# ishine/dmel_codec

Measured on AMD Instinct MI355X. Metric: audio-sec/sec (encode+decode RTF) @24 kHz batch 32, higher is better.
Workload: dtype f32; 1 GPU; cfg2: encode+decode, 24000 Hz, 80 mel, 8 FSQ groups [7, 5, 5], WaveNet 20+20 layers, BigVGAN-base, batch 32 x 1 s per GPU; lanes=3, vocoder_streams=1

## Files before the change

### dmel_codec_amd/csrc/conv_igemm.hip

```cpp
#include "conv.h"
#include "conv_dev.h"
#include "ops.h"
#include <type_traits>

#include <cmath>
#include <cstdlib>

namespace dmel {


template <int WAVES_M, int WAVES_N, int MT, int NT, int MODE, int HALO>
__global__ __launch_bounds__(64 * WAVES_M * WAVES_N) void conv_igemm_kernel(KArgs a) {
  constexpr int BM = WAVES_M * MT * 32, BN = WAVES_N * NT * 32, NW = WAVES_M * WAVES_N;
  constexpr int XS = BN + HALO;
  constexpr int RW = (kCK + NW - 1) / NW;
  constexpr int XC = (XS + 63) / 64;
  extern __shared__ __attribute__((aligned(16))) float smem[];
  float* Xs = smem;

  const int tid = threadIdx.x, lane = tid & 63, wave = tid >> 6;
  const int wave_m = wave / WAVES_N, wave_n = wave % WAVES_N;
  const int h = lane >> 5, l31 = lane & 31;
  int tile_n, mblk, b;
  if (!conv_block_coords(a, tile_n, mblk, b)) return;
  const int q0 = tile_n * BN;
  const int lb = b / a.len_div;

  floatx16 acc[MT][NT];
#pragma unroll
  for (int mi = 0; mi < MT; ++mi)
#pragma unroll
    for (int ni = 0; ni < NT; ++ni)
#pragma unroll
      for (int r = 0; r < 16; ++r) acc[mi][ni][r] = 0.f;

  const float4* wA[MT];
#pragma unroll
  for (int mi = 0; mi < MT; ++mi) {
    const int tile = min(mblk * (BM / 32) + wave_m * MT + mi, a.mtiles - 1);
    wA[mi] = reinterpret_cast<const float4*>(a.w) + (size_t)tile * a.steps * 128 + lane;
  }
  float4 ac0[MT], ac1[MT], an0[MT], an1[MT];
  float xr[RW][XC];

  auto load_x = [&](int sg, int chunk) {
    const float* xb = a.seg[sg].x + (int64_t)b * a.seg[sg].bstride;
    const int taps = a.seg[sg].taps, dil = a.seg[sg].dil, tstride = a.seg[sg].tstride, Cin = a.seg[sg].Cin;
    const int wx = BN + (taps - 1) * dil;
    const int tin = (int)a.seg[sg].Tin;
    const int lim = a.seg[sg].in_len ? min((int)min(a.seg[sg].in_len[lb], (int64_t)tin), tin) : tin;
    const int tau0 = q0 * tstride + a.seg[sg].toff - a.seg[sg].pad_left;
    const int cs = (int)a.seg[sg].cstride;
#pragma unroll
    for (int rr = 0; rr < RW; ++rr) {
      const int r = wave + rr * NW;
      const int ci = chunk * kCK + r;
      const bool rowok = (r < kCK) && (ci < Cin);
      const float* xrow = xb + min(ci, Cin - 1) * cs;
#pragma unroll
      for (int c = 0; c < XC; ++c) {
        const int j = lane + 64 * c;
        const int tau = tau0 + j * tstride;
        const bool ok = rowok && (j < wx) && (tau >= 0) && (tau < lim);
        const float v = xrow[min(max(tau, 0), tin - 1)];
        xr[rr][c] = ok ? v : 0.f;
      }
    }
  };
  auto store_x = [&](float* dst, float scale) {
#pragma unroll
    for (int rr = 0; rr < RW; ++rr) {
      const int r = wave + rr * NW;
#pragma unroll
      for (int c = 0; c < XC; ++c) {
        const int j = lane + 64 * c;
        if ((kCK % NW == 0 || r < kCK) && (XS % 64 == 0 || j < XS)) dst[r * XS + j] = xr[rr][c] * scale;
      }
    }
  };

  int sg = 0, chunk = 0, tap = 0, xbuf = 0;
  load_x(0, 0);
#pragma unroll
  for (int mi = 0; mi < MT; ++mi) { ac0[mi] = wA[mi][0]; ac1[mi] = wA[mi][64]; }
  store_x(Xs, a.seg[0].in_scale);
  __syncthreads();

  for (int s = 0; s < a.steps; ++s) {
    int nsg = sg, nchunk = chunk, ntap = tap + 1;
    bool newx = false;
    if (ntap == a.seg[sg].taps) {
      ntap = 0;
      ++nchunk;
      newx = true;
      if (nchunk == a.seg[sg].nchunk) { nchunk = 0; ++nsg; }
    }
    const bool has_next = s + 1 < a.steps;
    if (has_next) {
#pragma unroll
      for (int mi = 0; mi < MT; ++mi) {
        an0[mi] = wA[mi][(size_t)(s + 1) * 128];
        an1[mi] = wA[mi][(size_t)(s + 1) * 128 + 64];
      }
      if (newx) load_x(nsg, nchunk);
    }
    {
      const float* xp = Xs + xbuf * (kCK * XS) + wave_n * (NT * 32) + l31 + tap * a.seg[sg].dil + h * XS;
#pragma unroll
      for (int kk = 0; kk < kCK / 2; ++kk) {
        float av[MT], bv[NT];
#pragma unroll
        for (int mi = 0; mi < MT; ++mi) {
          const float4 q = (kk < 4) ? ac0[mi] : ac1[mi];
          av[mi] = (kk & 3) == 0 ? q.x : (kk & 3) == 1 ? q.y : (kk & 3) == 2 ? q.z : q.w;
        }
#pragma unroll
        for (int ni = 0; ni < NT; ++ni) bv[ni] = xp[2 * kk * XS + ni * 32];
#pragma unroll
        for (int mi = 0; mi < MT; ++mi)
#pragma unroll
          for (int ni = 0; ni < NT; ++ni)
            acc[mi][ni] = __builtin_amdgcn_mfma_f32_32x32x2f32(av[mi], bv[ni], acc[mi][ni], 0, 0, 0);
      }
    }
    if (has_next) {
#pragma unroll
      for (int mi = 0; mi < MT; ++mi) { ac0[mi] = an0[mi]; ac1[mi] = an1[mi]; }
      if (newx) {
        store_x(Xs + (xbuf ^ 1) * (kCK * XS), a.seg[nsg].in_scale);
        __syncthreads();
        xbuf ^= 1;
      }
    }
    sg = nsg; chunk = nchunk; tap = ntap;
  }

  conv_epilogue<MT, NT, MODE>(a, acc, mblk * BM + wave_m * (MT * 32), q0 + wave_n * (NT * 32) + l31, b, lb, h);
}

template <int WAVES_M, int WAVES_N, int MT, int NT, int MODE>
__global__ __launch_bounds__(64 * WAVES_M * WAVES_N) void conv_direct_kernel(KArgs a) {
  constexpr int BM = WAVES_M * MT * 32, BN = WAVES_N * NT * 32;
  const int tid = threadIdx.x, lane = tid & 63, wave = tid >> 6;
  const int wave_m = wave / WAVES_N, wave_n = wave % WAVES_N;
  const int h = lane >> 5, l31 = lane & 31;
  int tile_n, mblk, b;
  if (!conv_block_coords(a, tile_n, mblk, b)) return;
  const int q0 = tile_n * BN;
  const int lb = b / a.len_div;

  floatx16 acc[MT][NT];
#pragma unroll
  for (int mi = 0; mi < MT; ++mi)
#pragma unroll
    for (int ni = 0; ni < NT; ++ni)
#pragma unroll
      for (int r = 0; r < 16; ++r) acc[mi][ni][r] = 0.f;

  const float4* wA[MT];
#pragma unroll
  for (int mi = 0; mi < MT; ++mi) {
    const int tile = min(mblk * (BM / 32) + wave_m * MT + mi, a.mtiles - 1);
    wA[mi] = reinterpret_cast<const float4*>(a.w) + (size_t)tile * a.steps * 128 + lane;
  }
  const int qcol = q0 + wave_n * (NT * 32) + l31;

  float4 ac0[MT], ac1[MT], an0[MT], an1[MT];
  float bc[NT][8], bn[NT][8];
  int sbase = 0;

  for (int sg = 0; sg < a.nseg; ++sg) {
    const SegArgs& sa = a.seg[sg];
    const float* xb = sa.x + (int64_t)b * sa.bstride;
    const int taps = sa.taps, dil = sa.dil, cin = sa.Cin, cs = (int)sa.cstride, tin = (int)sa.Tin;
    const int lim = sa.in_len ? min((int)min(sa.in_len[lb], (int64_t)tin), tin) : tin;
    const float scale = sa.in_scale;
    const int nst = sa.nchunk * taps;
    int tcol[NT];
#pragma unroll
    for (int ni = 0; ni < NT; ++ni) tcol[ni] = (qcol + ni * 32) * sa.tstride + sa.toff - sa.pad_left;
    int rowoff[8];

#define DMEL_DIRECT_LOAD(A0, A1, B, chunk, tap, gstep)                                                  \
    {                                                                                                   \
      _Pragma("unroll") for (int mi = 0; mi < MT; ++mi) {                                               \
        A0[mi] = wA[mi][(size_t)(gstep) * 128];                                                         \
        A1[mi] = wA[mi][(size_t)(gstep) * 128 + 64];                                                    \
      }                                                                                                 \
      if ((tap) == 0) {                                                                                 \
        _Pragma("unroll") for (int kk = 0; kk < 8; ++kk)                                                \
          rowoff[kk] = min((chunk) * kCK + 2 * kk + h, cin - 1) * cs;                                   \
      }                                                                                                 \
      _Pragma("unroll") for (int ni = 0; ni < NT; ++ni) {                                               \
        const int tau = tcol[ni] + (tap) * dil;                                                         \
        const bool ok = (tau >= 0) && (tau < lim);                                                      \
        const int tc = min(max(tau, 0), tin - 1);                                                       \
        _Pragma("unroll") for (int kk = 0; kk < 8; ++kk) {                                              \
          const float v = xb[rowoff[kk] + tc];                                                          \
          B[ni][kk] = ok ? v * scale : 0.f;                                                             \
        }                                                                                               \
      }                                                                                                 \
    }

    int chunk = 0, tap = 0;
    DMEL_DIRECT_LOAD(ac0, ac1, bc, 0, 0, sbase)
    for (int ls = 0; ls < nst; ++ls) {
      int ntap = tap + 1, nchunk = chunk;
      if (ntap == taps) { ntap = 0; ++nchunk; }
      const bool has_next = ls + 1 < nst;
      if (has_next) DMEL_DIRECT_LOAD(an0, an1, bn, nchunk, ntap, sbase + ls + 1)
#pragma unroll
      for (int kk = 0; kk < 8; ++kk) {
        float av[MT];
#pragma unroll
        for (int mi = 0; mi < MT; ++mi) {
          const float4 q = (kk < 4) ? ac0[mi] : ac1[mi];
          av[mi] = (kk & 3) == 0 ? q.x : (kk & 3) == 1 ? q.y : (kk & 3) == 2 ? q.z : q.w;
        }
#pragma unroll
        for (int mi = 0; mi < MT; ++mi)
#pragma unroll
          for (int ni = 0; ni < NT; ++ni)
            acc[mi][ni] = __builtin_amdgcn_mfma_f32_32x32x2f32(av[mi], bc[ni][kk], acc[mi][ni], 0, 0, 0);
      }
      if (has_next) {
#pragma unroll
        for (int mi = 0; mi < MT; ++mi) { ac0[mi] = an0[mi]; ac1[mi] = an1[mi]; }
#pragma unroll
        for (int ni = 0; ni < NT; ++ni)
#pragma unroll
          for (int kk = 0; kk < 8; ++kk) bc[ni][kk] = bn[ni][kk];
      }
      chunk = nchunk; tap = ntap;
    }
#undef DMEL_DIRECT_LOAD
    sbase += nst;
  }
  conv_epilogue<MT, NT, MODE>(a, acc, mblk * BM + wave_m * (MT * 32), qcol, b, lb, h);
}

static int conv_grid(KArgs& k, int gx, int gy, int gz, dim3& grid) {
  static int mode = [] { const char* e = getenv("DMEL_CONV_XCD"); return e ? atoi(e) : -1; }();
  k.gx = gx; k.gy = gy; k.gz = gz;
  const double weight_bytes = (double)k.mtiles * 32.0 * k.steps * kCK * 4.0;
  const bool want = mode == 1 || (mode == -1 && weight_bytes > 2.5e6 && gy >= 8);
  const int64_t total = (int64_t)gx * gy * gz;
  if (want && total < ((int64_t)1 << 30)) {
    k.xcd_chunk = (int)((total + 7) / 8);
    grid = dim3((unsigned)(k.xcd_chunk * 8));
    return DMEL_OK;
  }
  k.xcd_chunk = 0;
  if (gy > 65535 || gz > 65535) {
    set_error("conv_igemm: grid too large (mblocks %d, batch %d)", gy, gz);
    return DMEL_EINVAL;
  }
  grid = dim3((unsigned)gx, (unsigned)gy, (unsigned)gz);
  return DMEL_OK;
}

template <int WM, int WN, int MT, int NT, int MODE> static int launch_d(const KArgs& ka, int B, int mblocks, hipStream_t st) {
  constexpr int BN = WN * NT * 32;
  KArgs k2 = ka;
  dim3 grid;
  DMEL_TRY(conv_grid(k2, (int)((ka.Tcols + BN - 1) / BN), mblocks, B, grid));
  hipLaunchKernelGGL((conv_direct_kernel<WM, WN, MT, NT, MODE>), grid, dim3(64 * WM * WN), 0, st, k2);
  DMEL_HIP(hipGetLastError());
  return DMEL_OK;
}

template <int WM, int WN, int MT, int NT, int MODE, int HALO>
static int launch_h(const KArgs& ka, int B, int mblocks, hipStream_t st) {
  constexpr int BN = WN * NT * 32;
  const size_t lds = (size_t)(2 * kCK * (BN + HALO)) * sizeof(float);
  KArgs k2 = ka;
  dim3 grid;
  DMEL_TRY(conv_grid(k2, (int)((ka.Tcols + BN - 1) / BN), mblocks, B, grid));
  hipLaunchKernelGGL((conv_igemm_kernel<WM, WN, MT, NT, MODE, HALO>), grid, dim3(64 * WM * WN), lds, st, k2);
  DMEL_HIP(hipGetLastError());
  return DMEL_OK;
}

template <int WM, int WN, int MT, int NT, int MODE> static int launch_t(const KArgs& ka, int B, int mblocks, hipStream_t st) {
  int halo = 0;
  for (int s = 0; s < ka.nseg; ++s) halo = std::max(halo, (ka.seg[s].taps - 1) * ka.seg[s].dil);
  if (halo == 0) return launch_h<WM, WN, MT, NT, MODE, 0>(ka, B, mblocks, st);
  if (halo <= 16) return launch_h<WM, WN, MT, NT, MODE, 16>(ka, B, mblocks, st);
  return launch_h<WM, WN, MT, NT, MODE, 64>(ka, B, mblocks, st);
}

typedef __bf16 bf16x8 __attribute__((ext_vector_type(8)));
typedef _Float16 f16x8 __attribute__((ext_vector_type(8)));
typedef _Float16 f16x2 __attribute__((ext_vector_type(2)));
#ifndef DMEL_PD
#define DMEL_PD 2
#endif
#ifndef DMEL_EXP
#define DMEL_EXP 0
#endif
#ifndef DMEL_PD2
#define DMEL_PD2 2
#endif
#ifndef DMEL_XTOP
#define DMEL_XTOP 0
#endif
#ifndef DMEL_BPF
#define DMEL_BPF 0
#endif
#ifndef DMEL_KG2
#define DMEL_KG2 2
#endif

__device__ __forceinline__ uint32_t pack_hi16(float lo, float hi) {
  return __builtin_amdgcn_perm(__float_as_uint(hi), __float_as_uint(lo), 0x07060302u);
}

template <int WAVES_M, int WAVES_N, int MT, int NT, int MODE, int HALO, int NP, int KG, int PS = 0>
__global__ __launch_bounds__(64 * WAVES_M * WAVES_N, NP == 2 ? 2 : 1) void conv_bf16_kernel(KArgs a) {
  static_assert(PS == 0 || NP == 2, "pre-split inputs exist for the fp16 split only");
  constexpr int BM = WAVES_M * MT * 32, BN = WAVES_N * NT * 32;
  constexpr int XS = BN + HALO;
  constexpr int SUB = KG / 2;
  constexpr int NWV = WAVES_M * WAVES_N;
  static_assert(NWV % KG == 0 || KG % NWV == 0, "waves and staged channel groups must divide one another");
  constexpr int SEG = NWV >= KG ? NWV / KG : 1;
  constexpr int RPW = NWV >= KG ? 1 : KG / NWV;
  constexpr int SL = (XS + SEG - 1) / SEG;
  constexpr int NPASS = (SL + 63) / 64;
  constexpr int NIT = RPW * NPASS;
  constexpr int PSZ = KG * XS;
  extern __shared__ __attribute__((aligned(16))) float smem[];
#ifndef DMEL_CONV_LDS_PAD
#define DMEL_CONV_LDS_PAD 0
#endif
  constexpr int kLdsPad = ((size_t)2 * NP * KG * XS * 16 + 2 * DMEL_CONV_LDS_PAD <= 65536) ? DMEL_CONV_LDS_PAD : 0;
  uint4* Xb = reinterpret_cast<uint4*>(smem) + kLdsPad / 16;

  const int tid = threadIdx.x, lane = tid & 63, wave = tid >> 6;
  const int wave_m = wave / WAVES_N, wave_n = wave % WAVES_N;
  const int h = lane >> 5, l31 = lane & 31;
  int tile_n, mblk, b;
  if (!conv_block_coords(a, tile_n, mblk, b)) return;
  const int q0 = tile_n * BN;
  const int lb = b / a.len_div;

  floatx16 acc[MT][NT];
#pragma unroll
  for (int mi = 0; mi < MT; ++mi)
#pragma unroll
    for (int ni = 0; ni < NT; ++ni)
#pragma unroll
      for (int r = 0; r < 16; ++r) acc[mi][ni][r] = 0.f;
  floatx16 acl[NP == 2 ? MT : 1][NP == 2 ? NT : 1];
  if constexpr (NP == 2) {
#pragma unroll
    for (int mi = 0; mi < MT; ++mi)
#pragma unroll
      for (int ni = 0; ni < NT; ++ni)
#pragma unroll
        for (int r = 0; r < 16; ++r) acl[mi][ni][r] = 0.f;
  }

  const char* wT[MT];
#pragma unroll
  for (int mi = 0; mi < MT; ++mi) {
    const int tile = __builtin_amdgcn_readfirstlane(min(mblk * (BM / 32) + wave_m * MT + mi, a.mtiles - 1));
    wT[mi] = reinterpret_cast<const char*>(NP == 3 ? a.w48 : NP == 2 ? a.w32h : a.w16) + (size_t)tile * a.steps * (NP * 1024);
  }
  const uint32_t lane16 = lane * 16;
  auto load_w = [&](uint4 (&dst)[MT][NP], int step) {
#pragma unroll
    for (int mi = 0; mi < MT; ++mi) {
      const char* sp = wT[mi] + (size_t)step * (NP * 1024);
#pragma unroll
      for (int p = 0; p < NP; ++p) dst[mi][p] = *reinterpret_cast<const uint4*>(sp + p * 1024 + lane16);
    }
  };
  float xr[NIT][8];

  auto seg_limit = [&](int sg) {
    const int tin = (int)a.seg[sg].Tin;
    return a.seg[sg].in_len ? (int)min(a.seg[sg].in_len[lb], (int64_t)tin) : tin;
  };
  const int lim0 = seg_limit(0), lim1 = a.nseg > 1 ? seg_limit(1) : 0;
  float f16_in = kF16XScale, f16_out = 1.f;
  if (NP == 2 && a.seg[0].in_absmax) {
    const int e = min(max((int)(*a.seg[0].in_absmax >> 23) - 127, -100), 100);
    f16_in = __uint_as_float((uint32_t)(127 + 13 - e) << 23);
    f16_out = __uint_as_float((uint32_t)(127 - 13 + e) << 23) * (1.f / kF16WScale);
  }
  bool xok[NIT];
  const int wave_u = __builtin_amdgcn_readfirstlane(wave);
  const int st_kg0 = (wave_u / SEG) * RPW, st_j0 = (wave_u % SEG) * SL;
  auto load_x = [&](int sg, int chunk) {
    if constexpr (PS != 0) {
      const int taps = a.seg[sg].taps, dil = a.seg[sg].dil;
      const int wx = BN + (taps - 1) * dil;
      const int tin = (int)a.seg[sg].Tin, g8 = a.seg[sg].xp_g8;
      const int lim = sg == 0 ? lim0 : lim1;
      const int tau0 = q0 + a.seg[sg].toff - a.seg[sg].pad_left;
      const uint4* xpb = a.seg[sg].xp + (int64_t)b * g8 * tin;
#pragma unroll
      for (int rr = 0; rr < RPW; ++rr) {
        const int kgi = chunk * KG + st_kg0 + rr;
        const uint4* rowp = xpb + (int64_t)min(kgi, g8 - 1) * tin;
#pragma unroll
        for (int ps = 0; ps < NPASS; ++ps) {
          const int it = rr * NPASS + ps;
          const int j = min(st_j0 + ps * 64 + lane, XS - 1);
          const int tau = tau0 + j;
          xok[it] = (j < wx) && (tau >= 0) && (tau < lim) && (kgi < g8);
          const uint4* ptr = rowp + min(max(tau, 0), tin - 1);
          const uint4 hi = *ptr, lo = *(ptr + a.seg[sg].xp_plane);
          xr[it][0] = __uint_as_float(hi.x); xr[it][1] = __uint_as_float(hi.y); xr[it][2] = __uint_as_float(hi.z); xr[it][3] = __uint_as_float(hi.w);
          xr[it][4] = __uint_as_float(lo.x); xr[it][5] = __uint_as_float(lo.y); xr[it][6] = __uint_as_float(lo.z); xr[it][7] = __uint_as_float(lo.w);
        }
      }
      return;
    }
    const char* xb = reinterpret_cast<const char*>(a.seg[sg].x + (int64_t)b * a.seg[sg].bstride);
    const int taps = a.seg[sg].taps, dil = a.seg[sg].dil, tstride = a.seg[sg].tstride, Cin = a.seg[sg].Cin;
    const int wx = BN + (taps - 1) * dil;
    const int tin = (int)a.seg[sg].Tin;
    const int lim = sg == 0 ? lim0 : lim1;
    const int tau0 = q0 * tstride + a.seg[sg].toff - a.seg[sg].pad_left;
    const uint32_t cs4 = (uint32_t)a.seg[sg].cstride * 4u, last = (uint32_t)(Cin - 1) * cs4;
#pragma unroll
    for (int rr = 0; rr < RPW; ++rr) {
      uint32_t row = (uint32_t)(chunk * (KG * 8) + (st_kg0 + rr) * 8) * cs4;
      const char* rowp[8];
#pragma unroll
      for (int e = 0; e < 8; ++e, row += cs4) rowp[e] = xb + min(row, last);
#pragma unroll
      for (int ps = 0; ps < NPASS; ++ps) {
        const int it = rr * NPASS + ps;
        const int j = min(st_j0 + ps * 64 + lane, XS - 1);
        const int tau = tau0 + j * tstride;
        xok[it] = (j < wx) && (tau >= 0) && (tau < lim);
        const uint32_t col = (uint32_t)min(max(tau, 0), tin - 1) * 4u;
#pragma unroll
        for (int e = 0; e < 8; ++e) xr[it][e] = *reinterpret_cast<const float*>(rowp[e] + col);
      }
    }
  };
  auto store_x = [&](uint4* dst, int sg, int chunk) {
#pragma clang fp contract(off)
    if constexpr (PS != 0) {
#pragma unroll
      for (int it = 0; it < NIT; ++it) {
        const int rr = it / NPASS, ps = it % NPASS;
        const int jl = ps * 64 + lane;
        const int j = st_j0 + jl;
        if ((SL % 64 != 0 && jl >= SL) || (XS % SL != 0 && j >= XS)) continue;
        const int i = (st_kg0 + rr) * XS + j;
        const bool ok = xok[it];
        dst[i] = make_uint4(ok ? __float_as_uint(xr[it][0]) : 0u, ok ? __float_as_uint(xr[it][1]) : 0u, ok ? __float_as_uint(xr[it][2]) : 0u,
                            ok ? __float_as_uint(xr[it][3]) : 0u);
        dst[PSZ + i] = make_uint4(ok ? __float_as_uint(xr[it][4]) : 0u, ok ? __float_as_uint(xr[it][5]) : 0u, ok ? __float_as_uint(xr[it][6]) : 0u,
                                  ok ? __float_as_uint(xr[it][7]) : 0u);
      }
      return;
    }
    const float scale = NP == 2 ? a.seg[sg].in_scale * f16_in : a.seg[sg].in_scale;
    const int Cin = a.seg[sg].Cin;
#pragma unroll
    for (int it = 0; it < NIT; ++it) {
      const int rr = it / NPASS, ps = it % NPASS;
      const int jl = ps * 64 + lane;
      const int j = st_j0 + jl;
      if ((SL % 64 != 0 && jl >= SL) || (XS % SL != 0 && j >= XS)) continue;
      const int i = (st_kg0 + rr) * XS + j;
      const int c0 = chunk * (KG * 8) + (st_kg0 + rr) * 8;
      float v[8];
#pragma unroll
      for (int e = 0; e < 8; ++e) v[e] = (xok[it] ? xr[it][e] : 0.f) * (c0 + e < Cin ? scale : 0.f);
      if constexpr (NP == 1) {
        bf16x8 p;
#pragma unroll
        for (int e = 0; e < 8; ++e) p[e] = (__bf16)v[e];
        dst[i] = __builtin_bit_cast(uint4, p);
      } else if constexpr (NP == 2) {
        f16x8 ph, pl;
#pragma unroll
        for (int e = 0; e < 8; e += 2) {
          typedef float f32x2 __attribute__((ext_vector_type(2)));
          const f16x2 hi = __builtin_convertvector((f32x2){v[e], v[e + 1]}, f16x2);
          const f16x2 lo = __builtin_convertvector((f32x2){(v[e] - (float)hi[0]) * kF16LoScale, (v[e + 1] - (float)hi[1]) * kF16LoScale}, f16x2);
          ph[e] = hi[0]; ph[e + 1] = hi[1];
          pl[e] = lo[0]; pl[e + 1] = lo[1];
        }
        dst[i] = __builtin_bit_cast(uint4, ph);
        dst[PSZ + i] = __builtin_bit_cast(uint4, pl);
      } else {
        uint32_t p1[4], p2[4], p3[4];
#pragma unroll
        for (int e = 0; e < 8; e += 2) {
          const float r0 = v[e] - __uint_as_float(__float_as_uint(v[e]) & 0xffff0000u);
          const float r1 = v[e + 1] - __uint_as_float(__float_as_uint(v[e + 1]) & 0xffff0000u);
          const float s0 = r0 - __uint_as_float(__float_as_uint(r0) & 0xffff0000u);
          const float s1 = r1 - __uint_as_float(__float_as_uint(r1) & 0xffff0000u);
          p1[e >> 1] = pack_hi16(v[e], v[e + 1]);
          p2[e >> 1] = pack_hi16(r0, r1);
          p3[e >> 1] = pack_hi16(s0, s1);
        }
        dst[i] = make_uint4(p1[0], p1[1], p1[2], p1[3]);
        dst[PSZ + i] = make_uint4(p2[0], p2[1], p2[2], p2[3]);
        dst[2 * PSZ + i] = make_uint4(p3[0], p3[1], p3[2], p3[3]);
      }
    }
  };
  int cur_taps = a.seg[0].taps, cur_nchunk = a.seg[0].nchunk, cur_dil = a.seg[0].dil;
  auto next_chunk = [&](int sg, int ck, int& nsg, int& nck) -> bool {
    nsg = sg; nck = ck + 1;
    if (nck * SUB >= cur_nchunk) { nck = 0; ++nsg; }
    return nsg < a.nseg;
  };

  int sg = 0, c16 = 0, tap = 0, xbuf = 0;
  int psg = 0, pck = 0;
  bool pending = false;
  constexpr int PD = NP == 2 ? DMEL_PD2 : DMEL_PD;
  uint4 wa[PD + 1][MT][NP];
#pragma unroll
  for (int d = 0; d < PD; ++d) load_w(wa[d], min(d, a.steps - 1));
  load_x(0, 0);
  store_x(Xb, 0, 0);
  __builtin_amdgcn_s_waitcnt(0x0f70);
  __syncthreads();
  int cstep = 0;

  constexpr int kWLoads = MT * NP;
  constexpr int kWKeep = (PD - 1) * kWLoads < 63 ? (PD - 1) * kWLoads : 63;
  constexpr int kWaitW = (kWKeep & 15) | (7 << 4) | (15 << 8) | ((kWKeep >> 4) << 14);
  constexpr int kXLoads = NIT * (PS != 0 ? 2 : 8);
  constexpr int kWX = kWKeep + kXLoads < 63 ? kWKeep + kXLoads : 63;
  [[maybe_unused]] constexpr int kWaitWX = (kWX & 15) | (7 << 4) | (15 << 8) | ((kWX >> 4) << 14);
#if DMEL_BPF
  bf16x8 bfrag[2][NT][NP];
  bool have_frag = false;
#endif
  auto k_step = [&](auto R, int s) {
    constexpr int r = decltype(R)::value;
    uint4 (&use)[MT][NP] = wa[r % (PD + 1)];
    int nsg = sg, nc16 = c16, ntap = tap + 1;
    bool newx = false;
    if (ntap == cur_taps) {
      ntap = 0;
      ++nc16;
      if (nc16 == cur_nchunk) { nc16 = 0; ++nsg; newx = true; }
      else newx = (nc16 % SUB) == 0;
    }
    const bool has_next = s + 1 < a.steps;
#if DMEL_XTOP
    bool x_younger = false;
    if (cstep == 0) {
      pending = next_chunk(sg, c16 / SUB, psg, pck);
      if (pending && !(DMEL_EXP & 2)) { load_x(psg, pck); x_younger = !newx; }
      if (DMEL_EXP & 2) pending = false;
    }
#endif
    if (!(DMEL_EXP & 4)) load_w(wa[(r + PD) % (PD + 1)], min(s + PD, a.steps - 1));
    {
#if DMEL_BPF
      bf16x8 (&bcur)[NT][NP] = bfrag[r % 2];
      bf16x8 (&bnxt)[NT][NP] = bfrag[(r + 1) % 2];
      if (!have_frag) {
        const uint4* xp = Xb + xbuf * (NP * PSZ) + ((c16 % SUB) * 2 + h) * XS + wave_n * (NT * 32) + l31 + tap * cur_dil;
#pragma unroll
        for (int ni = 0; ni < NT; ++ni)
#pragma unroll
          for (int p = 0; p < NP; ++p) bcur[ni][p] = __builtin_bit_cast(bf16x8, xp[p * PSZ + ni * 32]);
      }
      have_frag = has_next && !newx;
      if (have_frag) {
        const uint4* xq = Xb + xbuf * (NP * PSZ) + ((nc16 % SUB) * 2 + h) * XS + wave_n * (NT * 32) + l31 + ntap * cur_dil;
#pragma unroll
        for (int ni = 0; ni < NT; ++ni)
#pragma unroll
          for (int p = 0; p < NP; ++p) bnxt[ni][p] = __builtin_bit_cast(bf16x8, xq[p * PSZ + ni * 32]);
      }
#else
      const uint4* xp = Xb + xbuf * (NP * PSZ) + ((c16 % SUB) * 2 + h) * XS + wave_n * (NT * 32) + l31 + tap * cur_dil;
      bf16x8 bcur[NT][NP];
#pragma unroll
      for (int ni = 0; ni < NT; ++ni)
#pragma unroll
        for (int p = 0; p < NP; ++p) bcur[ni][p] = __builtin_bit_cast(bf16x8, xp[p * PSZ + ni * 32]);
#endif
      if constexpr (NP == 2) {
#pragma unroll
        for (int mi = 0; mi < MT; ++mi)
#pragma unroll
          for (int ni = 0; ni < NT; ++ni) {
            const f16x8 ah = __builtin_bit_cast(f16x8, use[mi][0]), al = __builtin_bit_cast(f16x8, use[mi][1]);
            const f16x8 bh = __builtin_bit_cast(f16x8, bcur[ni][0]), bl = __builtin_bit_cast(f16x8, bcur[ni][1]);
            acl[mi][ni] = __builtin_amdgcn_mfma_f32_32x32x16_f16(ah, bl, acl[mi][ni], 0, 0, 0);
            acl[mi][ni] = __builtin_amdgcn_mfma_f32_32x32x16_f16(al, bh, acl[mi][ni], 0, 0, 0);
            acc[mi][ni] = __builtin_amdgcn_mfma_f32_32x32x16_f16(ah, bh, acc[mi][ni], 0, 0, 0);
          }
      } else {
        constexpr int PA[6] = {2, 1, 0, 1, 0, 0}, PB[6] = {0, 1, 2, 0, 1, 0};
#pragma unroll
        for (int t = 0; t < (NP == 3 ? 6 : 1); ++t)
#pragma unroll
          for (int mi = 0; mi < MT; ++mi)
#pragma unroll
            for (int ni = 0; ni < NT; ++ni)
              acc[mi][ni] = __builtin_amdgcn_mfma_f32_32x32x16_bf16(__builtin_bit_cast(bf16x8, use[mi][NP == 3 ? PA[t] : 0]),
                                                                    bcur[ni][NP == 3 ? PB[t] : 0], acc[mi][ni], 0, 0, 0);
      }
    }
#if DMEL_XTOP
    if (x_younger) __builtin_amdgcn_s_waitcnt(kWaitWX);
    else __builtin_amdgcn_s_waitcnt(kWaitW);
#else
    __builtin_amdgcn_s_waitcnt(kWaitW);
    if (cstep == 0) {
      pending = next_chunk(sg, c16 / SUB, psg, pck);
      if (pending && !(DMEL_EXP & 2)) load_x(psg, pck);
      if (DMEL_EXP & 2) pending = false;
    }
#endif
    if (pending && (((DMEL_EXP & 1) ? false : cstep == 1) || newx)) {
      store_x(Xb + (xbuf ^ 1) * (NP * PSZ), psg, pck);
      pending = false;
    }
    ++cstep;
    if (has_next && newx) {
      __syncthreads();
      xbuf ^= 1;
      cstep = 0;
      if (nsg != sg) { cur_taps = a.seg[nsg].taps; cur_nchunk = a.seg[nsg].nchunk; cur_dil = a.seg[nsg].dil; }
    }
    sg = nsg; c16 = nc16; tap = ntap;
  };
  constexpr int UNR = DMEL_BPF ? ((PD + 1) % 2 ? 2 * (PD + 1) : PD + 1) : PD + 1;
  static_assert(UNR <= 8, "k_step calls below cover an unroll of up to eight");
  for (int s = 0; s < a.steps; s += UNR) {
    k_step(std::integral_constant<int, 0>{}, s);
    if (s + 1 < a.steps) k_step(std::integral_constant<int, 1>{}, s + 1);
    if (UNR > 2 && s + 2 < a.steps) k_step(std::integral_constant<int, 2 % UNR>{}, s + 2);
    if (UNR > 3 && s + 3 < a.steps) k_step(std::integral_constant<int, 3 % UNR>{}, s + 3);
    if (UNR > 4 && s + 4 < a.steps) k_step(std::integral_constant<int, 4 % UNR>{}, s + 4);
    if (UNR > 5 && s + 5 < a.steps) k_step(std::integral_constant<int, 5 % UNR>{}, s + 5);
    if (UNR > 6 && s + 6 < a.steps) k_step(std::integral_constant<int, 6 % UNR>{}, s + 6);
    if (UNR > 7 && s + 7 < a.steps) k_step(std::integral_constant<int, 7 % UNR>{}, s + 7);
  }
  if constexpr (NP == 2) {
#pragma unroll
    for (int mi = 0; mi < MT; ++mi)
#pragma unroll
      for (int ni = 0; ni < NT; ++ni)
#pragma unroll
        for (int r = 0; r < 16; ++r) acc[mi][ni][r] = fmaf(acl[mi][ni][r], 1.f / kF16LoScale, acc[mi][ni][r]) * f16_out;
  }
  if ((DMEL_EXP & 8) && acc[0][0][0] != 12345.f) return;
  conv_epilogue<MT, NT, MODE, NP == 2 ? 8 : 4>(a, acc, mblk * BM + wave_m * (MT * 32), q0 + wave_n * (NT * 32) + l31, b, lb, h);
}

template <int WM, int WN, int MT, int NT, int MODE, int HALO, int NP, int KG, int PS = 0>
static int launch_b16k(const KArgs& ka, int B, int mblocks, hipStream_t st) {
  constexpr int BN = WN * NT * 32;
#ifndef DMEL_CONV_LDS_PAD
#define DMEL_CONV_LDS_PAD 0
#endif
  constexpr size_t lds0 = (size_t)2 * NP * KG * (BN + HALO) * 16;
  constexpr size_t lds = lds0 + (lds0 + 2 * DMEL_CONV_LDS_PAD <= 65536 ? 2 * DMEL_CONV_LDS_PAD : 0);
  static_assert(lds <= 64 * 1024, "bf16 conv tile exceeds the default dynamic LDS limit");
  KArgs k2 = ka;
  dim3 grid;
  DMEL_TRY(conv_grid(k2, (int)((ka.Tcols + BN - 1) / BN), mblocks, B, grid));
  hipLaunchKernelGGL((conv_bf16_kernel<WM, WN, MT, NT, MODE, HALO, NP, KG, PS>), grid, dim3(64 * WM * WN), lds, st, k2);
  DMEL_HIP(hipGetLastError());
  return DMEL_OK;
}

template <int WM, int WN, int MT, int NT, int MODE, int NP> static int launch_b16(const KArgs& ka, int B, int mblocks, hipStream_t st) {
  int halo = 0;
  for (int s = 0; s < ka.nseg; ++s) halo = std::max(halo, (ka.seg[s].taps - 1) * ka.seg[s].dil);
  constexpr int KG0 = (WN * NT * 32 >= 256 && NP == 3) ? 2 : 4;
  if (halo == 0) return launch_b16k<WM, WN, MT, NT, MODE, 0, NP, KG0>(ka, B, mblocks, st);
  constexpr int KGT = (NP == 2 && 2 * NP * DMEL_KG2 * (WN * NT * 32 + 64) * 16 <= 65536) ? DMEL_KG2 : 2;
  if (halo <= 16) return launch_b16k<WM, WN, MT, NT, MODE, 16, NP, KGT>(ka, B, mblocks, st);
  return launch_b16k<WM, WN, MT, NT, MODE, 64, NP, KGT>(ka, B, mblocks, st);
}

#ifndef DMEL_TILE5_NARROW
#define DMEL_TILE5_NARROW 1
#endif
template <int MODE, int NP> static int launch_mode_bf16(const KArgs& ka, int tile, int B, hipStream_t st) {
  const int bm[8] = {128, 128, 64, 32, 128, DMEL_TILE5_NARROW ? 128 : 64, 128, 256};
  const int mblocks = (ka.mtiles * 32 + bm[tile] - 1) / bm[tile];
  switch (tile) {
    case 0: return launch_b16<2, 2, 2, 2, MODE, NP>(ka, B, mblocks, st);
    case 1: return launch_b16<4, 1, 1, 3, MODE, NP>(ka, B, mblocks, st);
    case 2: return launch_b16<2, 2, 1, 2, MODE, NP>(ka, B, mblocks, st);
    case 3: return launch_b16<1, 4, 1, 2, MODE, NP>(ka, B, mblocks, st);
    case 4: return launch_b16<4, 1, 1, 4, MODE, NP>(ka, B, mblocks, st);
    case 6: return launch_b16<4, 1, 1, 2, MODE, NP>(ka, B, mblocks, st);
    case 7: return launch_b16<8, 1, 1, 3, MODE, NP>(ka, B, mblocks, st);
#if DMEL_TILE5_NARROW
    default: return launch_b16<4, 1, 1, 1, MODE, NP>(ka, B, mblocks, st);
#else
    default: return launch_b16<2, 1, 1, 4, MODE, NP>(ka, B, mblocks, st);
#endif
  }
}

static int pick_tile_bf16(int mtiles, int64_t T, int np, int steps, int B) {
  const char* e = getenv("DMEL_CONV_TILE_BF16");
  const int forced = (e && e[0]) ? atoi(e) : -1;
  if (forced >= 0 && forced < 8) return forced;
  int t;
  if (np == 2 && mtiles >= 8 && T > 96) t = 7;
  else if (np == 2 && mtiles >= 4 && mtiles < 8 && steps >= 40) t = 6;
  else if (mtiles >= 4) t = (T > 2048 && np != 2) ? 4 : 1;
  else if (mtiles >= 2) t = 2;
  else t = 3;
  if (np == 2 && mtiles >= 4) {
    static const int bm[8] = {128, 128, 64, 32, 128, DMEL_TILE5_NARROW ? 128 : 64, 128, 256};
    static const int bn[8] = {128, 96, 128, 256, 128, DMEL_TILE5_NARROW ? 32 : 128, 64, 96};
    auto wgs = [&](int tt) { return (int64_t)((mtiles * 32 + bm[tt] - 1) / bm[tt]) * ((T + bn[tt] - 1) / bn[tt]) * B; };
    static const bool off = [] { const char* f = getenv("DMEL_CONV_SMALLN"); return f && f[0] == '0'; }();
    if (!off && wgs(t) < 128) {
      t = 6;
      if (DMEL_TILE5_NARROW && wgs(6) < 128) t = 5;
    }
  }
  return t;
}

template <int MODE> static int launch_presplit(const KArgs& ka, int B, int64_t Tcols, hipStream_t st) {
  int halo = 0;
  for (int s = 0; s < ka.nseg; ++s) halo = std::max(halo, (ka.seg[s].taps - 1) * ka.seg[s].dil);
  if (halo > 16) { set_error("conv (pre-split input): receptive field %d exceeds the 16-column halo built for this path", halo); return DMEL_EUNSUPPORTED; }
  const bool wide = ka.mtiles >= 8 && Tcols > 96;
  if (wide) {
    const int mblocks = (ka.mtiles * 32 + 255) / 256;
    if (halo == 0) return launch_b16k<8, 1, 1, 3, MODE, 0, 2, 4, 1>(ka, B, mblocks, st);
    return launch_b16k<8, 1, 1, 3, MODE, 16, 2, DMEL_KG2, 1>(ka, B, mblocks, st);
  }
  const int mblocks = (ka.mtiles * 32 + 127) / 128;
  if (halo == 0) return launch_b16k<4, 1, 1, 3, MODE, 0, 2, 4, 1>(ka, B, mblocks, st);
  return launch_b16k<4, 1, 1, 3, MODE, 16, 2, DMEL_KG2, 1>(ka, B, mblocks, st);
}

template <int NP> static int launch_bf16_any(const KArgs& ka, EpiMode mode, int B, int64_t Tcols, hipStream_t st) {
  const int t16 = pick_tile_bf16(ka.mtiles, Tcols, NP, ka.steps, B);
  switch (mode) {
    case EPI_LINEAR: return launch_mode_bf16<EPI_LINEAR, NP>(ka, t16, B, st);
    case EPI_GATE: return launch_mode_bf16<EPI_GATE, NP>(ka, t16, B, st);
    default: return launch_mode_bf16<EPI_RESSKIP, NP>(ka, t16, B, st);
  }
}

struct TileCfg {
  int wm, wn, mt, nt;
  float eff;
};
static const TileCfg kTiles[] = {
    {2, 2, 2, 2, 0.93f},
    {4, 1, 1, 3, 1.00f},
    {2, 2, 1, 2, 0.92f},
    {2, 1, 1, 3, 0.85f},
    {1, 4, 1, 2, 0.90f},
    {1, 4, 1, 1, 0.80f},
    {1, 3, 1, 1, 0.80f},
    {1, 4, 1, 1, 0.00f},
    {1, 3, 1, 1, 0.00f},
    {1, 4, 1, 2, 0.00f},
    {2, 2, 1, 2, 0.00f},
    {4, 1, 1, 3, 0.00f},
    {2, 2, 2, 2, 0.00f},
    {2, 2, 1, 1, 0.00f},
};
constexpr int kNumTiles = sizeof(kTiles) / sizeof(kTiles[0]);

static int pick_tile(int mtiles, int64_t T, int B) {
  static int forced = [] {
    const char* e = getenv("DMEL_CONV_TILE");
    return e ? atoi(e) : -1;
  }();
  if (forced >= 0 && forced < kNumTiles) return forced;
  if (T <= 96 && mtiles >= 4) return 8;
  int best = 0;
  double best_cost = 1e300;
  for (int i = 0; i < kNumTiles; ++i) {
    if (kTiles[i].eff <= 0.f) continue;
    const int bm = kTiles[i].wm * kTiles[i].mt * 32, bn = kTiles[i].wn * kTiles[i].nt * 32;
    const double wgs = (double)((mtiles * 32 + bm - 1) / bm) * (double)((T + bn - 1) / bn) * B;
    const double rounds = std::ceil(wgs / 256.0);
    const double cost = (wgs > 1024 ? wgs / 256.0 : rounds) * bm * bn / kTiles[i].eff;
    if (cost < best_cost) { best_cost = cost; best = i; }
  }
  return best;
}

template <int MODE> static int launch_mode(const KArgs& ka, int tile, int B, hipStream_t st) {
  const TileCfg& t = kTiles[tile];
  const int mblocks = (ka.mtiles * 32 + t.wm * t.mt * 32 - 1) / (t.wm * t.mt * 32);
  switch (tile) {
    case 0: return launch_t<2, 2, 2, 2, MODE>(ka, B, mblocks, st);
    case 1: return launch_t<4, 1, 1, 3, MODE>(ka, B, mblocks, st);
    case 2: return launch_t<2, 2, 1, 2, MODE>(ka, B, mblocks, st);
    case 3: return launch_t<2, 1, 1, 3, MODE>(ka, B, mblocks, st);
    case 4: return launch_t<1, 4, 1, 2, MODE>(ka, B, mblocks, st);
    case 5: return launch_t<1, 4, 1, 1, MODE>(ka, B, mblocks, st);
    case 6: return launch_t<1, 3, 1, 1, MODE>(ka, B, mblocks, st);
    case 7: return launch_d<1, 4, 1, 1, MODE>(ka, B, mblocks, st);
    case 8: return launch_d<1, 3, 1, 1, MODE>(ka, B, mblocks, st);
    case 9: return launch_d<1, 4, 1, 2, MODE>(ka, B, mblocks, st);
    case 10: return launch_d<2, 2, 1, 2, MODE>(ka, B, mblocks, st);
    case 11: return launch_d<4, 1, 1, 3, MODE>(ka, B, mblocks, st);
    case 12: return launch_d<2, 2, 2, 2, MODE>(ka, B, mblocks, st);
    default: return launch_d<2, 2, 1, 1, MODE>(ka, B, mblocks, st);
  }
}

__global__ __launch_bounds__(256) void split_planes_kernel(const float* __restrict__ x, uint4* __restrict__ planes, int64_t plane_units,
                                                           const int64_t* __restrict__ len, int len_div, int C, int T) {
  const int b = blockIdx.z, g = blockIdx.y;
  const int t = blockIdx.x * 256 + threadIdx.x;
  if (t >= T) return;
  const float* xr = x + ((int64_t)b * C + g * 8) * T + t;
  const bool live = !len || t < len[b / len_div];
  float v[8];
#pragma unroll
  for (int e = 0; e < 8; ++e) v[e] = live ? xr[(int64_t)e * T] : 0.f;
  f16x8 ph, pl;
  {
#pragma clang fp contract(off)
#pragma unroll
    for (int e = 0; e < 8; e += 2) {
      typedef float f32x2 __attribute__((ext_vector_type(2)));
      const float s0 = v[e] * kF16XScale, s1 = v[e + 1] * kF16XScale;
      const f16x2 hi = __builtin_convertvector((f32x2){s0, s1}, f16x2);
      const f16x2 lo = __builtin_convertvector((f32x2){(s0 - (float)hi[0]) * kF16LoScale, (s1 - (float)hi[1]) * kF16LoScale}, f16x2);
      ph[e] = hi[0]; ph[e + 1] = hi[1];
      pl[e] = lo[0]; pl[e + 1] = lo[1];
    }
  }
  const int64_t i = ((int64_t)b * (C / 8) + g) * T + t;
  planes[i] = __builtin_bit_cast(uint4, ph);
  planes[plane_units + i] = __builtin_bit_cast(uint4, pl);
}
int launch_split_planes(const float* x, void* planes, int64_t plane_units, const int64_t* len, int len_div, int B, int C, int64_t T,
                        hipStream_t stream) {
  DMEL_CHECK_ARG(x && planes && B > 0 && B <= 65535 && C > 0 && C % 8 == 0 && C / 8 <= 65535 && T > 0 && T < ((int64_t)1 << 30), "split_planes: bad argument");
  ProfScope ps("small", stream, 0.0, 8.0 * B * C * (double)T);
  hipLaunchKernelGGL(split_planes_kernel, dim3((unsigned)((T + 255) / 256), (unsigned)(C / 8), (unsigned)B), dim3(256), 0, stream, x,
                     reinterpret_cast<uint4*>(planes), plane_units, len, len_div > 0 ? len_div : 1, C, (int)T);
  DMEL_HIP(hipGetLastError());
  return DMEL_OK;
}

static int check_f16_range(const PackedConv& pc, const ConvRun& r, hipStream_t stream) {
  static const int range_check = [] { const char* e = getenv("DMEL_DEBUG_F16_RANGE"); return e ? atoi(e) : 0; }();
  if (!range_check) return DMEL_OK;
  const PackDesc& d = pc.d;
  for (int s = 0; s < d.nseg; ++s) {
    const SegRun& sr = r.seg[s];
    if (sr.in_absmax || sr.cstride != sr.Tin || sr.bstride != (int64_t)d.seg[s].Cin * sr.cstride) continue;
    const uint32_t* slot = nullptr;
    DMEL_TRY(launch_absmax(sr.x, (int64_t)r.B * sr.bstride, stream, &slot));
    uint32_t bits = 0;
    DMEL_HIP(hipMemcpyAsync(&bits, slot, sizeof(bits), hipMemcpyDeviceToHost, stream));
    DMEL_HIP(hipStreamSynchronize(stream));
    float mx;
    std::memcpy(&mx, &bits, sizeof(mx));
    if (!(mx * sr.in_scale < kF16WScale * 65504.f)) {
      set_error("conv (fp16 split): max |x| = %g of input segment %d is outside the documented domain |x| < %g "
                "(DMEL_PRECISION_FP32_F16X2; use DMEL_PRECISION_FP32_BF16X3 for such tensors)", (double)mx * sr.in_scale, s,
                (double)(kF16WScale * 65504.f));
      return DMEL_EINVAL;
    }
  }
  return DMEL_OK;
}

int launch_conv(const PackedConv& pc, const ConvRun& r, hipStream_t stream) {
  {
    const char* e = getenv("DMEL_CONV_PC");
    if (!(e && e[0] == '0') && conv_pc_eligible(pc, r, e && e[0] == '2')) {
      DMEL_TRY(check_f16_range(pc, r, stream));
      return launch_conv_pc(pc, r, stream);
    }
  }
  KArgs ka{};
  const PackDesc& d = pc.d;
  ka.nseg = d.nseg;
  ka.steps = pc.steps;
  int max_halo = 0;
  for (int s = 0; s < d.nseg; ++s) {
    const SegDesc& sd = d.seg[s];
    SegArgs& o = ka.seg[s];
    DMEL_CHECK_ARG(r.seg[s].x != nullptr || r.seg[s].xp != nullptr, "conv: input pointer of segment %d is NULL", s);
    DMEL_CHECK_ARG(r.seg[s].xp == nullptr || (r.precision == DMEL_PRECISION_FP32_F16X2 && sd.Cin % 8 == 0 && sd.tstride == 1 &&
                                              r.seg[s].in_scale == 1.f && r.seg[s].tshift == 0 && r.seg[s].in_absmax == nullptr && r.fold_pitch == 0),
                   "conv: a pre-split input needs the fp16-split precision, channels %% 8 == 0, unit stride and scale");
    DMEL_CHECK_ARG((r.seg[s].xp != nullptr) == (r.seg[0].xp != nullptr), "conv: either every input segment is pre-split or none is");
    DMEL_CHECK_ARG(sd.taps == 1 || sd.tstride == 1 || (r.precision != DMEL_PRECISION_FP32_MFMA && !getenv("DMEL_CONV_FP32_MFMA")),
                   "conv: taps>1 with strided input is unsupported by the native fp32-MFMA kernel");
    o.x = r.seg[s].x; o.bstride = r.seg[s].bstride; o.cstride = r.seg[s].cstride; o.Tin = r.seg[s].Tin;
    o.in_len = r.seg[s].in_len; o.in_scale = r.seg[s].in_scale;
    o.in_absmax = (s == 0 && d.nseg == 1 && r.precision == DMEL_PRECISION_FP32_F16X2) ? r.seg[s].in_absmax : nullptr;
    o.xp = reinterpret_cast<const uint4*>(r.seg[s].xp); o.xp_plane = r.seg[s].xp_plane; o.xp_g8 = sd.Cin / 8;
    o.Cin = sd.Cin; o.nchunk = (sd.Cin + kCK - 1) / kCK; o.taps = sd.taps; o.dil = sd.dil;
    o.pad_left = sd.pad_left; o.tstride = sd.tstride; o.toff = sd.toff + (int)(r.seg[s].tshift * sd.tstride);
    max_halo = std::max(max_halo, (sd.taps - 1) * sd.dil);
    DMEL_CHECK_ARG((int64_t)sd.Cin * o.cstride < ((int64_t)1 << 30) && o.Tin * sd.tstride < ((int64_t)1 << 30),
                   "conv: one batch item of the input exceeds 32-bit byte offsets (4 GiB)");
  }
  if (max_halo > 64) {
    set_error("conv_igemm: receptive field (taps-1)*dilation = %d exceeds the 64-sample LDS halo", max_halo);
    return DMEL_EUNSUPPORTED;
  }
  DMEL_CHECK_ARG(r.y != nullptr && r.B > 0 && r.Tcols > 0, "conv: bad output/batch/length");
  DMEL_CHECK_ARG(d.mode != EPI_RESSKIP || r.skip != nullptr, "conv: skip buffer missing");
  ka.w = pc.w.as<float>(); ka.w16 = pc.w16.p; ka.w48 = pc.w48.p; ka.w32h = pc.w32h.p; ka.bias = pc.bias.as<float>();
  ka.Tcols = r.Tcols; ka.mode = d.mode; ka.act = r.act; ka.C = d.C; ka.RP = pc.RP; ka.phases = d.phases;
  ka.out_tstride = r.out_tstride; ka.phase_base = r.phase_base; ka.accumulate = r.accumulate;
  ka.len_div = r.len_div > 0 ? r.len_div : 1; ka.skip_first = r.skip_first; ka.out_div = r.out_div;
  ka.y = r.y; ka.y_bs = r.y_bs; ka.y_cs = r.y_cs; ka.Tout = r.Tout > 0 ? r.Tout : r.Tcols * r.out_tstride;
  ka.res = r.res; ka.res_bs = r.res_bs; ka.res_cs = r.res_cs; ka.row_scale = r.row_scale;
  ka.out_len = r.out_len; ka.skip = r.skip;
  ka.fold_pitch = r.fold_pitch; ka.fold_valid = r.fold_valid;
  DMEL_CHECK_ARG(r.yp == nullptr || (d.mode != EPI_LINEAR && d.C % 8 == 0 && r.out_tstride == 1), "conv: pre-split output needs a paired mode and C %% 8 == 0");
  ka.yp = reinterpret_cast<uint4*>(r.yp); ka.yp_plane = r.yp_plane; ka.yp_g8 = d.C / 8; ka.yp_only = r.yp_only;
  DMEL_CHECK_ARG(r.fold_pitch == 0 || (r.fold_pitch >= r.fold_valid && r.fold_valid > 0 && r.B == 1 && r.out_tstride == 1),
                 "conv: folded-batch launches are single-item, unit-stride and need 0 < fold_valid <= fold_pitch");
  DMEL_CHECK_ARG((int64_t)d.C * ka.y_cs < ((int64_t)1 << 31) && ka.Tout < ((int64_t)1 << 30) && ka.Tcols < ((int64_t)1 << 30),
                 "conv: one batch item of the output exceeds 32-bit offsets");
  ka.mtiles = pc.Mpad / 32;
  const double rows_real = (d.mode == EPI_LINEAR ? (double)d.C * d.phases : 2.0 * d.C);
  double in_elems = 0.0;
  for (int s = 0; s < d.nseg; ++s) in_elems += (double)d.seg[s].Cin * (double)std::min<int64_t>(r.seg[s].Tin, r.Tcols * d.seg[s].tstride + max_halo);
  double out_elems;
  if (d.mode == EPI_LINEAR) out_elems = (double)d.C * d.phases * (double)r.Tcols * (1.0 + (r.res ? 1.0 : 0.0) + (r.accumulate ? 1.0 : 0.0));
  else if (d.mode == EPI_GATE) out_elems = (double)d.C * (double)r.Tcols;
  else out_elems = (double)d.C * (double)r.Tcols * (r.skip_first ? 3.0 : 4.0);
  double alg_bytes = 4.0 * r.B * (in_elems + out_elems);
  static const int native_fp32 = [] { const char* e = getenv("DMEL_CONV_FP32_MFMA"); return e ? atoi(e) : 0; }();
  const bool one_piece = r.precision == DMEL_PRECISION_BF16 || train_precision_override() == DMEL_PRECISION_BF16;
  const bool native = !one_piece && (native_fp32 || r.precision == DMEL_PRECISION_FP32_MFMA);
  const double products = one_piece ? 1.0 : native ? 16.0  : r.precision == DMEL_PRECISION_FP32_F16X2 ? 3.0 : 6.0;
  alg_bytes += (double)pc.Mpad * pc.steps * kCK * (one_piece ? 2.0 : native ? 4.0 : r.precision == DMEL_PRECISION_FP32_F16X2 ? 4.0 : 6.0);
  const double alg_flops = 2.0 * r.B * (double)r.Tcols * rows_real * pc.k_real;
  ProfScope ps("conv_igemm", stream, alg_flops, alg_bytes, alg_flops * products);
  if (r.precision == DMEL_PRECISION_BF16 || train_precision_override() == DMEL_PRECISION_BF16)
    return launch_bf16_any<1>(ka, d.mode, r.B, r.Tcols, stream);
  if (r.seg[0].xp != nullptr) {
    DMEL_CHECK_ARG(!native_fp32 && train_precision_override() != DMEL_PRECISION_BF16 && d.mode != EPI_LINEAR,
                   "conv: pre-split inputs are built for the paired modes of the fp16-split kernel");
    return d.mode == EPI_GATE ? launch_presplit<EPI_GATE>(ka, r.B, r.Tcols, stream) : launch_presplit<EPI_RESSKIP>(ka, r.B, r.Tcols, stream);
  }
  if (r.precision == DMEL_PRECISION_FP32_F16X2 && !native_fp32) {
    DMEL_TRY(check_f16_range(pc, r, stream));
    return launch_bf16_any<2>(ka, d.mode, r.B, r.Tcols, stream);
  }
  if ((r.precision == DMEL_PRECISION_FP32 || r.precision == DMEL_PRECISION_FP32_BF16X3 || r.precision == DMEL_PRECISION_FP32_F16X2) && !native_fp32)
    return launch_bf16_any<3>(ka, d.mode, r.B, r.Tcols, stream);
  const int tile = pick_tile(ka.mtiles, r.Tcols, r.B);
  switch (d.mode) {
    case EPI_LINEAR: return launch_mode<EPI_LINEAR>(ka, tile, r.B, stream);
    case EPI_GATE: return launch_mode<EPI_GATE>(ka, tile, r.B, stream);
    default: return launch_mode<EPI_RESSKIP>(ka, tile, r.B, stream);
  }
}

}

using namespace dmel;


extern "C" int dmel_conv_set_precision(dmel_conv* c, int precision) {
  DMEL_CHECK_ARG(c && valid_precision(precision), "conv_set_precision: not a DMEL_PRECISION_* value");
  c->precision = precision;
  return DMEL_OK;
}

extern "C" int dmel_conv_create(dmel_conv** out, const float* w_host, const float* bias_host, int Cout, int Cin, int k,
                                int dilation) {
  DMEL_CHECK_ARG(out && w_host, "NULL argument");
  DMEL_CHECK_ARG(Cout > 0 && Cin > 0 && k > 0 && (k % 2) == 1 && dilation > 0, "conv: bad shape (odd k required)");
  auto* c = new dmel_conv();
  c->Cout = Cout; c->Cin = Cin; c->k = k; c->dil = dilation;
  PackDesc d;
  d.mode = EPI_LINEAR; d.nseg = 1; d.C = Cout; d.phases = 1;
  d.seg[0].Cin = Cin; d.seg[0].taps = k; d.seg[0].dil = dilation; d.seg[0].pad_left = dilation * (k - 1) / 2;
  int rc = pack_conv(c->pc, d,
                     [&](int, int row, int ci, int tap) { return w_host[((size_t)row * Cin + ci) * k + tap]; },
                     [&](int row) { return bias_host ? bias_host[row] : 0.f; });
  if (rc != DMEL_OK) { delete c; return rc; }
  c->w_host.assign(w_host, w_host + (size_t)Cout * Cin * k);
  *out = c;
  return DMEL_OK;
}

extern "C" void dmel_conv_destroy(dmel_conv* c) { delete c; }

extern "C" int dmel_conv_forward(const dmel_conv* c, const float* x, float* y, int B, int64_t T, void* stream) {
  DMEL_CHECK_ARG(c && x && y, "NULL argument");
  ConvRun r;
  r.seg[0].x = x; r.seg[0].bstride = (int64_t)c->Cin * T; r.seg[0].cstride = T; r.seg[0].Tin = T;
  r.B = B; r.Tcols = T; r.y = y; r.y_bs = (int64_t)c->Cout * T; r.y_cs = T; r.Tout = T;
  r.precision = c->precision;
  return launch_conv(c->pc, r, (hipStream_t)stream);
}
```

Measured before the change: 2408 audio-sec/sec.

## Specialize bf16 conv K loop on compile-time tap count for single-segment convs

Adds a TAPS template parameter and a dedicated K loop for single-segment, stride-1 convolutions in the fp16-split path. Tap and sub-channel offsets become compile-time constants, and the X prefetch/store/sync happen at fixed points within each chunk. This replaces the generic per-step bookkeeping (segment/chunk/tap advancement and branches). The cost is more template instantiations and code size, plus a new schedule for overlapping loads with compute; an env var can disable it.

```diff
diff --git a/dmel_codec_amd/csrc/conv_igemm.hip b/dmel_codec_amd/csrc/conv_igemm.hip
--- a/dmel_codec_amd/csrc/conv_igemm.hip
+++ b/dmel_codec_amd/csrc/conv_igemm.hip
@@ -1,7 +1,9 @@
 #include "conv.h"
 #include "conv_dev.h"
 #include "ops.h"
+#include <numeric>
 #include <type_traits>
+#include <utility>
 
 #include <cmath>
 #include <cstdlib>
@@ -315,9 +317,15 @@
   return __builtin_amdgcn_perm(__float_as_uint(hi), __float_as_uint(lo), 0x07060302u);
 }
 
-template <int WAVES_M, int WAVES_N, int MT, int NT, int MODE, int HALO, int NP, int KG, int PS = 0>
+template <class F, int... I> __device__ __forceinline__ void static_for_impl(F& f, std::integer_sequence<int, I...>) {
+  (f(std::integral_constant<int, I>{}), ...);
+}
+template <int N, class F> __device__ __forceinline__ void static_for(F&& f) { static_for_impl(f, std::make_integer_sequence<int, N>{}); }
+
+template <int WAVES_M, int WAVES_N, int MT, int NT, int MODE, int HALO, int NP, int KG, int PS = 0, int TAPS = 0>
 __global__ __launch_bounds__(64 * WAVES_M * WAVES_N, NP == 2 ? 2 : 1) void conv_bf16_kernel(KArgs a) {
   static_assert(PS == 0 || NP == 2, "pre-split inputs exist for the fp16 split only");
+  static_assert(TAPS == 0 || (NP == 2 && PS == 0), "the single-segment K loop is built for the fp16 split of fp32 inputs");
   constexpr int BM = WAVES_M * MT * 32, BN = WAVES_N * NT * 32;
   constexpr int XS = BN + HALO;
   constexpr int SUB = KG / 2;
@@ -634,17 +642,76 @@
     }
     sg = nsg; c16 = nc16; tap = ntap;
   };
-  constexpr int UNR = DMEL_BPF ? ((PD + 1) % 2 ? 2 * (PD + 1) : PD + 1) : PD + 1;
-  static_assert(UNR <= 8, "k_step calls below cover an unroll of up to eight");
-  for (int s = 0; s < a.steps; s += UNR) {
-    k_step(std::integral_constant<int, 0>{}, s);
-    if (s + 1 < a.steps) k_step(std::integral_constant<int, 1>{}, s + 1);
-    if (UNR > 2 && s + 2 < a.steps) k_step(std::integral_constant<int, 2 % UNR>{}, s + 2);
-    if (UNR > 3 && s + 3 < a.steps) k_step(std::integral_constant<int, 3 % UNR>{}, s + 3);
-    if (UNR > 4 && s + 4 < a.steps) k_step(std::integral_constant<int, 4 % UNR>{}, s + 4);
-    if (UNR > 5 && s + 5 < a.steps) k_step(std::integral_constant<int, 5 % UNR>{}, s + 5);
-    if (UNR > 6 && s + 6 < a.steps) k_step(std::integral_constant<int, 6 % UNR>{}, s + 6);
-    if (UNR > 7 && s + 7 < a.steps) k_step(std::integral_constant<int, 7 % UNR>{}, s + 7);
+  if constexpr (TAPS > 0) {
+    constexpr int SPC = SUB * TAPS;
+    constexpr int CU = (PD + 1) / std::gcd(SPC, PD + 1);
+    const int nck = a.steps / SPC;
+    const int last = a.steps - 1, dil = cur_dil;
+    const uint4* xl = Xb + h * XS + wave_n * (NT * 32) + l31;
+    auto chunk_steps = [&](auto U, int c) {
+      const bool more = c + 1 < nck;
+      const uint4* xc = xl + xbuf * (NP * PSZ);
+      static_for<SPC>([&](auto J) {
+        constexpr int j = decltype(J)::value, r = (decltype(U)::value * SPC + j) % (PD + 1);
+        constexpr int sub = j / TAPS, tap = j % TAPS;
+        if (!(DMEL_EXP & 4)) load_w(wa[(r + PD) % (PD + 1)], min(c * SPC + (j + PD), last));
+        const uint4* xp = xc + sub * 2 * XS + tap * dil;
+        bf16x8 bcur[NT][NP];
+#pragma unroll
+        for (int ni = 0; ni < NT; ++ni)
+#pragma unroll
+          for (int p = 0; p < NP; ++p) bcur[ni][p] = __builtin_bit_cast(bf16x8, xp[p * PSZ + ni * 32]);
+#pragma unroll
+        for (int mi = 0; mi < MT; ++mi)
+#pragma unroll
+          for (int ni = 0; ni < NT; ++ni) {
+            const f16x8 ah = __builtin_bit_cast(f16x8, wa[r][mi][0]), al = __builtin_bit_cast(f16x8, wa[r][mi][1]);
+            const f16x8 bh = __builtin_bit_cast(f16x8, bcur[ni][0]), bl = __builtin_bit_cast(f16x8, bcur[ni][1]);
+            acl[mi][ni] = __builtin_amdgcn_mfma_f32_32x32x16_f16(ah, bl, acl[mi][ni], 0, 0, 0);
+            acl[mi][ni] = __builtin_amdgcn_mfma_f32_32x32x16_f16(al, bh, acl[mi][ni], 0, 0, 0);
+            acc[mi][ni] = __builtin_amdgcn_mfma_f32_32x32x16_f16(ah, bh, acc[mi][ni], 0, 0, 0);
+          }
+        __builtin_amdgcn_s_waitcnt(kWaitW);
+        if constexpr (j == 0) {
+          if (more && !(DMEL_EXP & 2)) load_x(0, c + 1);
+        }
+        if constexpr (j == (SPC > 1 ? 1 : 0)) {
+          if (more && !(DMEL_EXP & 2)) store_x(Xb + (xbuf ^ 1) * (NP * PSZ), 0, c + 1);
+        }
+        if constexpr (j == SPC - 1) {
+          if (more) {
+            __syncthreads();
+            xbuf ^= 1;
+          }
+        }
+      });
+    };
+    static_assert(CU <= 3, "the chunk group below covers up to three chunks");
+    for (int c = 0;; c += CU) {
+      chunk_steps(std::integral_constant<int, 0>{}, c);
+      if (c + 1 >= nck) break;
+      if constexpr (CU > 1) {
+        chunk_steps(std::integral_constant<int, 1>{}, c + 1);
+        if (c + 2 >= nck) break;
+      }
+      if constexpr (CU > 2) {
+        chunk_steps(std::integral_constant<int, 2>{}, c + 2);
+        if (c + 3 >= nck) break;
+      }
+    }
+  } else {
+    constexpr int UNR = DMEL_BPF ? ((PD + 1) % 2 ? 2 * (PD + 1) : PD + 1) : PD + 1;
+    static_assert(UNR <= 8, "k_step calls below cover an unroll of up to eight");
+    for (int s = 0; s < a.steps; s += UNR) {
+      k_step(std::integral_constant<int, 0>{}, s);
+      if (s + 1 < a.steps) k_step(std::integral_constant<int, 1>{}, s + 1);
+      if (UNR > 2 && s + 2 < a.steps) k_step(std::integral_constant<int, 2 % UNR>{}, s + 2);
+      if (UNR > 3 && s + 3 < a.steps) k_step(std::integral_constant<int, 3 % UNR>{}, s + 3);
+      if (UNR > 4 && s + 4 < a.steps) k_step(std::integral_constant<int, 4 % UNR>{}, s + 4);
+      if (UNR > 5 && s + 5 < a.steps) k_step(std::integral_constant<int, 5 % UNR>{}, s + 5);
+      if (UNR > 6 && s + 6 < a.steps) k_step(std::integral_constant<int, 6 % UNR>{}, s + 6);
+      if (UNR > 7 && s + 7 < a.steps) k_step(std::integral_constant<int, 7 % UNR>{}, s + 7);
+    }
   }
   if constexpr (NP == 2) {
 #pragma unroll
@@ -658,7 +725,7 @@
   conv_epilogue<MT, NT, MODE, NP == 2 ? 8 : 4>(a, acc, mblk * BM + wave_m * (MT * 32), q0 + wave_n * (NT * 32) + l31, b, lb, h);
 }
 
-template <int WM, int WN, int MT, int NT, int MODE, int HALO, int NP, int KG, int PS = 0>
+template <int WM, int WN, int MT, int NT, int MODE, int HALO, int NP, int KG, int PS = 0, int TAPS = 0>
 static int launch_b16k(const KArgs& ka, int B, int mblocks, hipStream_t st) {
   constexpr int BN = WN * NT * 32;
 #ifndef DMEL_CONV_LDS_PAD
@@ -670,17 +737,57 @@
   KArgs k2 = ka;
   dim3 grid;
   DMEL_TRY(conv_grid(k2, (int)((ka.Tcols + BN - 1) / BN), mblocks, B, grid));
-  hipLaunchKernelGGL((conv_bf16_kernel<WM, WN, MT, NT, MODE, HALO, NP, KG, PS>), grid, dim3(64 * WM * WN), lds, st, k2);
+  hipLaunchKernelGGL((conv_bf16_kernel<WM, WN, MT, NT, MODE, HALO, NP, KG, PS, TAPS>), grid, dim3(64 * WM * WN), lds, st, k2);
   DMEL_HIP(hipGetLastError());
   return DMEL_OK;
+}
+
+static bool conv_spec_enabled() {
+  const char* e = getenv("DMEL_CONV_SPEC");
+  return !(e && e[0] == '0');
+}
+
+template <int WM, int WN, int MT, int NT, int MODE, int KG0, int KGT>
+static bool launch_spec(const KArgs& ka, int halo, int B, int mblocks, hipStream_t st, int& rc) {
+  constexpr bool amp = MODE == EPI_LINEAR && MT == 1 && ((WM == 4 && WN == 1 && (NT == 2 || NT == 3)) || (WM == 2 && WN == 2 && NT == 2) ||
+                                                         (WM == 1 && WN == 4 && NT == 2) || (WM == 8 && WN == 1 && NT == 3));
+  constexpr bool amp64 = amp && NT == 2;
+  constexpr bool pw = MODE != EPI_GATE && WM == 4 && WN == 1 && MT == 1 && NT == 3;
+  if constexpr (amp || pw) {
+    const SegArgs& sa = ka.seg[0];
+    if (ka.nseg != 1 || sa.tstride != 1 || sa.xp != nullptr || !conv_spec_enabled()) return false;
+    const int taps = sa.taps, sub = halo == 0 ? KG0 / 2 : KGT / 2;
+    if (sa.nchunk % sub != 0 || ka.steps != sa.nchunk * taps) return false;
+    if constexpr (amp) {
+      if (halo > 0 && halo <= 16) {
+        if (taps == 3) { rc = launch_b16k<WM, WN, MT, NT, MODE, 16, 2, KGT, 0, 3>(ka, B, mblocks, st); return true; }
+        if (taps == 7) { rc = launch_b16k<WM, WN, MT, NT, MODE, 16, 2, KGT, 0, 7>(ka, B, mblocks, st); return true; }
+        if (taps == 11) { rc = launch_b16k<WM, WN, MT, NT, MODE, 16, 2, KGT, 0, 11>(ka, B, mblocks, st); return true; }
+      }
+      if constexpr (amp64) {
+        if (halo > 16) {
+          if (taps == 7) { rc = launch_b16k<WM, WN, MT, NT, MODE, 64, 2, KGT, 0, 7>(ka, B, mblocks, st); return true; }
+          if (taps == 11) { rc = launch_b16k<WM, WN, MT, NT, MODE, 64, 2, KGT, 0, 11>(ka, B, mblocks, st); return true; }
+        }
+      }
+    }
+    if constexpr (pw) {
+      if (halo == 0) { rc = launch_b16k<WM, WN, MT, NT, MODE, 0, 2, KG0, 0, 1>(ka, B, mblocks, st); return true; }
+    }
+  }
+  return false;
 }
 
 template <int WM, int WN, int MT, int NT, int MODE, int NP> static int launch_b16(const KArgs& ka, int B, int mblocks, hipStream_t st) {
   int halo = 0;
   for (int s = 0; s < ka.nseg; ++s) halo = std::max(halo, (ka.seg[s].taps - 1) * ka.seg[s].dil);
   constexpr int KG0 = (WN * NT * 32 >= 256 && NP == 3) ? 2 : 4;
+  constexpr int KGT = (NP == 2 && 2 * NP * DMEL_KG2 * (WN * NT * 32 + 64) * 16 <= 65536) ? DMEL_KG2 : 2;
+  if constexpr (NP == 2) {
+    int rc = DMEL_OK;
+    if (launch_spec<WM, WN, MT, NT, MODE, KG0, KGT>(ka, halo, B, mblocks, st, rc)) return rc;
+  }
   if (halo == 0) return launch_b16k<WM, WN, MT, NT, MODE, 0, NP, KG0>(ka, B, mblocks, st);
-  constexpr int KGT = (NP == 2 && 2 * NP * DMEL_KG2 * (WN * NT * 32 + 64) * 16 <= 65536) ? DMEL_KG2 : 2;
   if (halo <= 16) return launch_b16k<WM, WN, MT, NT, MODE, 16, NP, KGT>(ka, B, mblocks, st);
   return launch_b16k<WM, WN, MT, NT, MODE, 64, NP, KGT>(ka, B, mblocks, st);
 }
```

Result: faster. 2460 audio-sec/sec (median of 6 runs) (+2.2%).
